# alessandroragano/nomad

Hardware: NVIDIA B200
Metric: utterance-seconds embedded per second (higher is better)
Workload: dtype fp16

## Files before the change

### nomad_b200/csrc/gemm.cu

```cuda
#include "gemm.cuh"

#include <cmath>
#include <cstdlib>
#include <cstring>
#include <mutex>
#include <vector>

namespace nb {

static constexpr int BM = 128;
static constexpr int BK = 64;
static constexpr int UMMA_K = 16;
static constexpr int NUM_EPI_WARPS = 8;
static constexpr int GEMM_THREADS = 128 + NUM_EPI_WARPS * 32;
static constexpr float CD_REFINE = 1e-3f;

template <int BN>
struct TileCfg {
    static constexpr int A_BYTES = BM * BK * 2;
    static constexpr int B_BYTES = BN * BK * 2;
    static constexpr int STAGE_BYTES = A_BYTES + B_BYTES;
    static constexpr int STAGES = (BN == 256) ? 4 : (BN == 192 ? 4 : (BN == 128 ? 5 : 7));
    static constexpr int ACC_STRIDE = BN <= 64 ? 64 : (BN <= 128 ? 128 : 256);
    static constexpr int TMEM_COLS = 2 * ACC_STRIDE;
    static constexpr int EPI_STAGE_BYTES = NUM_EPI_WARPS * 4096;
    static constexpr int SMEM_BYTES = STAGES * STAGE_BYTES + EPI_STAGE_BYTES + 1024  + 256 ;
};

struct GemmArgs {
    int M, N, K, batch;
    int umma_n;
    int m_tiles, n_tiles;
    int a_wrap;
    int shared_ab, b_kshift0, b_kshift_step, b_mod;
    int resid_tma;
    int resid_l2pf;
    unsigned sleep_ns;
    GemmEpilogue epi;
};
__device__ __forceinline__ void mbar_wait_role(uint64_t* bar, uint32_t parity, unsigned ns) {
    if (mbar_try_wait(bar, parity)) return;
    while (!mbar_try_wait(bar, parity))
        if (ns) __nanosleep(ns);
}

struct RowCtx {
    float2 st;
    float pm, pM2;
    float* rbuf;
    bool rhave;
    const float* rnext;
    const CUtensorMap* tm_r;
    uint64_t* rbar;
    uint32_t rphase;
    const float* rbase;
    const float* vec;
    int vec_stride;
    int vec_col0;
    const CUtensorMap* tm_f;
    const CUtensorMap* tm_h;
    const CUtensorMap* tm_a;
    uint32_t pending;
    int stage_bytes;
    int flip;
};
__device__ __forceinline__ void resid_tma_issue(const CUtensorMap* map, uint64_t* bar, float* rbuf, const float* src,
                                                const float* base, long long ld, int lane) {
    if (lane == 0) {
        const long long off = src - base;
        const int row = (int)(off / ld), col = (int)(off - (long long)row * ld);
        mbar_expect_tx(bar, 4096);
        tma_load_2d_cta(rbuf, map, bar, col, row);
    }
}
__device__ __forceinline__ void ts_acquire(RowCtx& rc, uint32_t mask, int lane) {
    if (rc.pending & mask) {
        if (lane == 0) bulk_wait_read();
        rc.pending = 0;
    }
    __syncwarp();
    rc.pending |= mask;
}
__device__ __forceinline__ void ts_issue(const CUtensorMap* map, const void* src, int col, long long row, int lane) {
    fence_proxy_async_smem();
    __syncwarp();
    if (lane == 0) {
        tma_store_2d(map, src, col, (int)row);
        bulk_commit();
    }
}
__device__ __forceinline__ int ts_h16_slot(RowCtx& rc, bool f32_too) {
    if (rc.stage_bytes >= 6144) return 4096;
    if (f32_too) return 0;
    rc.flip ^= 1;
    return rc.flip * 2048;
}
__device__ __forceinline__ float2 ln_row_stats(const float* part, long long row) {
    const float4* p = reinterpret_cast<const float4*>(part + row * (2 * LN_PARTS));
    float m[LN_PARTS], M2 = 0.f, mean = 0.f;
#pragma unroll
    for (int i = 0; i < LN_PARTS / 2; ++i) {
        const float4 t = __ldg(p + i);
        m[2 * i] = t.x; m[2 * i + 1] = t.z;
        M2 += t.y + t.w;
        mean += t.x + t.z;
    }
    mean *= 1.0f / LN_PARTS;
    float d2 = 0.f;
#pragma unroll
    for (int i = 0; i < LN_PARTS; ++i) d2 = fmaf(m[i] - mean, m[i] - mean, d2);
    const float var = fmaf(64.0f, d2, M2) * (1.0f / (64.0f * LN_PARTS));
    return make_float2(mean, rsqrtf(var + 1e-5f));
}

template <int EF>
__device__ __forceinline__ int epi_flags(const GemmEpilogue& e) { return EF >= 0 ? EF : e.flags; }

template <int EF>
__device__ __forceinline__ float2 epilogue_row_stats(const GemmArgs& args, long long row) {
    if (row >= args.M || !(epi_flags<EF>(args.epi) & (EPI_LN_FOLD | EPI_RESID_LN))) return make_float2(0.f, 1.f);
    return args.epi.ln_part != nullptr ? ln_row_stats(args.epi.ln_part, row)
                                       : __ldg(reinterpret_cast<const float2*>(args.epi.ln_stats) + row);
}

template <int EF, int W>
__device__ __forceinline__ void epilogue_stage_vectors(const GemmEpilogue& e, float* vec, int c0, int lane) {
    const int flags = epi_flags<EF>(e);
    __syncwarp();
    if (lane * 4 < W) {
        if (flags & EPI_BIAS) reinterpret_cast<float4*>(vec)[lane] = __ldg(reinterpret_cast<const float4*>(e.bias + c0) + lane);
        if (flags & EPI_LN_FOLD) {
            reinterpret_cast<float4*>(vec)[lane] = __ldg(reinterpret_cast<const float4*>(e.fold_c + c0) + lane);
            reinterpret_cast<float4*>(vec + W)[lane] = __ldg(reinterpret_cast<const float4*>(e.fold_s + c0) + lane);
        }
        if (flags & EPI_RESID_LN) {
            reinterpret_cast<float4*>(vec + W)[lane] = __ldg(reinterpret_cast<const float4*>(e.ln_g + c0) + lane);
            reinterpret_cast<float4*>(vec + 2 * W)[lane] = __ldg(reinterpret_cast<const float4*>(e.ln_b + c0) + lane);
        }
    }
    __syncwarp();
}

template <bool FULL, int EF, bool PREC = false, bool TS = false, bool SV = false, bool RP = false>
__device__ __forceinline__ void epilogue_chunk(const GemmEpilogue& e, float (&v)[32], long long row, bool row_ok,
                                               int rows_valid, int col0, int ncols, int b, float* stage, int lane,
                                               RowCtx& rc) {
    const int flags = epi_flags<EF>(e);
    const long long off = row * e.ldo + col0 + (long long)b * e.out_bstride;
    const long long woff = (row - lane) * e.ldo + col0 + (long long)b * e.out_bstride;
    if (PREC) {
        const float sc = e.acc_scale;
#pragma unroll
        for (int j = 0; j < 32; ++j) v[j] *= sc;
    }
    if ((FULL || row_ok) && (flags & EPI_BIAS)) {
        const float4* bp = reinterpret_cast<const float4*>(e.bias + (long long)b * e.bias_bstride + col0);
#pragma unroll
        for (int j = 0; j < 8; ++j) {
            if (FULL || j * 4 < ncols) {
                const float4 t = (FULL && (SV || rc.vec)) ? *reinterpret_cast<const float4*>(rc.vec + (col0 - rc.vec_col0) + 4 * j)
                                                          : __ldg(bp + j);
                v[4 * j + 0] += t.x; v[4 * j + 1] += t.y; v[4 * j + 2] += t.z; v[4 * j + 3] += t.w;
            }
        }
    }
    if ((FULL || row_ok) && (flags & EPI_LN_FOLD)) {
        const float4* sp = reinterpret_cast<const float4*>(e.fold_s + col0);
        const float4* cp = reinterpret_cast<const float4*>(e.fold_c + col0);
        const float nm = -rc.st.x, rs = rc.st.y;
#pragma unroll
        for (int j = 0; j < 8; ++j) {
            if (FULL || j * 4 < ncols) {
                const bool sv = FULL && (SV || rc.vec != nullptr);
                const float4 a = sv ? *reinterpret_cast<const float4*>(rc.vec + rc.vec_stride + (col0 - rc.vec_col0) + 4 * j)
                                    : __ldg(sp + j);
                const float4 c = sv ? *reinterpret_cast<const float4*>(rc.vec + (col0 - rc.vec_col0) + 4 * j) : __ldg(cp + j);
#if NB_F32X2
                const float2 nm2 = make_float2(nm, nm), rs2 = make_float2(rs, rs);
                const float2 lo = ffma2(rs2, ffma2(nm2, make_float2(a.x, a.y), make_float2(v[4 * j + 0], v[4 * j + 1])), make_float2(c.x, c.y));
                const float2 hi = ffma2(rs2, ffma2(nm2, make_float2(a.z, a.w), make_float2(v[4 * j + 2], v[4 * j + 3])), make_float2(c.z, c.w));
                v[4 * j + 0] = lo.x; v[4 * j + 1] = lo.y; v[4 * j + 2] = hi.x; v[4 * j + 3] = hi.y;
#else
// ... 211 lines not shown
        for (int j = 0; j < 32; ++j) nbv[j] = j < ncols ? __ldg(e.norm_b + col0 + j) : 0.f;
    }
    const float m2s = -2.0f * e.cd_inv_scale;
    float dmin = CD_REFINE;
#pragma unroll
    for (int j = 0; j < 32; ++j) {
        v[j] = fmaf(v[j], m2s, na + nbv[j]);
        if (full || j < ncols) dmin = fminf(dmin, v[j]);
    }
    if (row_ok && dmin < CD_REFINE) {
#pragma unroll
        for (int j = 0; j < 32; ++j)
            if (j < ncols && v[j] < CD_REFINE) v[j] = cdist_exact_d2(e.cd_a + row * 256, e.cd_b + (long long)(col0 + j) * 256);
    }
    float s4[4] = {0.f, 0.f, 0.f, 0.f};
#pragma unroll
    for (int j = 0; j < 32; ++j) {
        v[j] = sqrt_approx(fmaxf(v[j], 0.f));
        if (full || j < ncols) s4[j & 3] += v[j];
    }
    s32 = (s4[0] + s4[1]) + (s4[2] + s4[3]);
    const double rs = row_ok ? (double)s32 : 0.0;
    if (e.out_f != nullptr && ts != nullptr && ts->tm_f != nullptr) {
        ts->flip ^= 1;
        float* sp = stage + (ts->stage_bytes >= 8192 ? ts->flip * 1024 : 0);
        ts_acquire(*ts, ts->stage_bytes >= 8192 ? (3u << (2 * ts->flip)) : 3u, lane);
        stage_put_f32(sp, v, lane);
        ts_issue(ts->tm_f, sp, col0, row - lane, lane);
    } else if (e.out_f != nullptr) {
        stage_put_f32(stage, v, lane);
        float* wout = e.out_f + (row - lane) * e.ldo + col0;
        if (full && (e.ldo & 3) == 0 && ((reinterpret_cast<uintptr_t>(wout) & 15) == 0)) {
            stage_flush_f32(stage, wout, e.ldo, rows_valid, ncols, lane);
        } else {
            __syncwarp();
            for (int rl = 0; rl < 32 && rl < rows_valid; ++rl)
                if (lane < ncols) wout[rl * e.ldo + lane] = stage[rl * 32 + ((((lane >> 2) ^ (rl & 7)) << 2) | (lane & 3))];
            __syncwarp();
        }
    }
    return rs;
}

struct StoreMaps {
    const CUtensorMap *f, *h, *a;
    const CUtensorMap* r;
    uint64_t* rbar;
    uint32_t* rphase;
    int stage_bytes;
    uint32_t* pending;
    int* flip;
};

template <int CHUNKS, bool PAIR, bool CDIST, int EF, bool PREC = false, int PACC = 0, bool TS = false, bool SV = false, bool RP = false>
__device__ __forceinline__ void epilogue_tile(const GemmArgs& args, uint32_t taddr, long long row, int col_first,
                                              int ccol_first, int b, uint64_t* tmem_empty_bar, int lane, float* stage,
                                              float2 row_st, float* rbuf, bool& rhave, const float* next_tile_src,
                                              const float* vec = nullptr, int vec_stride = 0, int cd_group = 0,
                                              const StoreMaps* sm = nullptr) {
    const bool row_ok = row < args.M;
    const long long rv = (long long)args.M - (row - lane);
    const int rows_valid = rv > 32 ? 32 : (rv < 0 ? 0 : (int)rv);
    double row_sum = 0.0;
    RowCtx rc;
    rc.st = row_st;
    rc.pm = rc.pM2 = 0.f;
    rc.rbuf = rbuf;
    rc.rhave = rhave;
    rc.rnext = nullptr;
    rc.vec = vec;
    rc.vec_stride = vec_stride;
    rc.vec_col0 = col_first;
    rc.tm_f = rc.tm_h = rc.tm_a = nullptr;
    rc.tm_r = nullptr; rc.rbar = nullptr; rc.rphase = 0; rc.rbase = args.epi.resid;
    if (sm != nullptr && sm->r != nullptr) { rc.tm_r = sm->r; rc.rbar = sm->rbar; rc.rphase = *sm->rphase; }
    rc.pending = 0;
    rc.stage_bytes = 4096;
    rc.flip = 0;
    if (TS && sm != nullptr) {
        rc.tm_f = sm->f; rc.tm_h = sm->h; rc.tm_a = sm->a;
        rc.stage_bytes = sm->stage_bytes;
        rc.pending = *sm->pending;
        rc.flip = *sm->flip;
    }
#pragma unroll 1
    for (int c = 0; c < CHUNKS; ++c) {
        uint32_t r[32];
        tmem_ld_32x32(taddr + c * 32, r);
        tmem_ld_wait();
        if (PREC && PACC > 0) {
#pragma unroll 1
            for (int a = 1; a < 4; ++a) {
                uint32_t q[32];
                tmem_ld_32x32(taddr + a * PACC + c * 32, q);
                tmem_ld_wait();
#pragma unroll
                for (int j = 0; j < 32; ++j) r[j] = __float_as_uint(__uint_as_float(r[j]) + __uint_as_float(q[j]));
            }
        }
        if (c == CHUNKS - 1) {
            tc_fence_before();
            __syncwarp();
            if (lane == 0) {
                if (PAIR) mbar_arrive_cluster(tmem_empty_bar, 0); else mbar_arrive(tmem_empty_bar);
            }
        }
        const int col0 = col_first + c * 32;
        int ncols = args.N - col0;
        ncols = ncols > 32 ? 32 : ncols;
        if (ccol_first + c * 32 >= args.umma_n) ncols = 0;
        if (!CDIST && rbuf != nullptr) {
            rc.rnext = next_tile_src;
            if (c + 1 < CHUNKS) {
                const int col1 = col0 + 32;
                rc.rnext = (rows_valid == 32 && col1 + 32 <= args.N && ccol_first + (c + 1) * 32 + 32 <= args.umma_n)
                               ? args.epi.resid + (row - lane) * args.epi.ldr + col1
                               : nullptr;
            }
        }
        if (ncols > 0 && rows_valid > 0) {
            float v[32];
#pragma unroll
            for (int j = 0; j < 32; ++j) v[j] = __uint_as_float(r[j]);
            if (CDIST) row_sum += cdist_chunk(args.epi, v, row, row_ok, rows_valid, col0, ncols, stage, lane, TS ? &rc : nullptr);
            else if (rows_valid == 32 && ncols == 32) epilogue_chunk<true, EF, PREC, TS, SV, RP>(args.epi, v, row, true, 32, col0, 32, b, stage, lane, rc);
            else epilogue_chunk<false, EF, PREC, TS>(args.epi, v, row, row_ok, rows_valid, col0, ncols, b, stage, lane, rc);
        }
    }
    rhave = rc.rhave;
    if (sm != nullptr && sm->r != nullptr) *sm->rphase = rc.rphase;
    if (TS && sm != nullptr) {
        *sm->pending = rc.pending;
        *sm->flip = rc.flip;
    }
    if (CDIST && row_ok) args.epi.row_part[(long long)cd_group * args.M + row] = (float)row_sum;
}

template <int BN, bool CDIST, bool PREC = false>
__global__ void __launch_bounds__(GEMM_THREADS, 1)
gemm_tc_kernel(const __grid_constant__ CUtensorMap tmA, const __grid_constant__ CUtensorMap tmB,
               const __grid_constant__ CUtensorMap tmA2, const __grid_constant__ CUtensorMap tmB2, const GemmArgs args) {
    using Cfg = TileCfg<BN>;
    constexpr int STAGES = Cfg::STAGES;
    extern __shared__ uint8_t smem_raw[];
    uint8_t* smem = smem_raw + ((1024u - (smem_u32(smem_raw) & 1023u)) & 1023u);
    float* epi_stage = reinterpret_cast<float*>(smem + STAGES * Cfg::STAGE_BYTES);
    uint64_t* full_bar = reinterpret_cast<uint64_t*>(smem + STAGES * Cfg::STAGE_BYTES + Cfg::EPI_STAGE_BYTES);
    uint64_t* empty_bar = full_bar + STAGES;
    uint64_t* tmem_full = empty_bar + STAGES;
    uint64_t* tmem_empty = tmem_full + 2;
    uint32_t* tmem_slot = reinterpret_cast<uint32_t*>(tmem_empty + 2);

    const int warp = threadIdx.x >> 5;
    const int lane = threadIdx.x & 31;
    const int num_tiles = args.m_tiles * args.n_tiles * args.batch;
    const int k_blocks = (args.K + BK - 1) / BK;
    const int k_total = PREC ? 3 * k_blocks : k_blocks;

    if (warp == 0 && lane == 0) {
        tma_prefetch_desc(&tmA);
        tma_prefetch_desc(&tmB);
    }
    if (warp == 1 && lane == 0) {
        for (int s = 0; s < STAGES; ++s) {
            mbar_init(&full_bar[s], 1);
            mbar_init(&empty_bar[s], 1);
// ... 45 lines not shown
            }
        }
    } else if (warp == 1) {
        if (lane == 0) {
            const uint32_t idesc = umma_idesc_h16(BM, args.umma_n);
            int stage = 0;
            uint32_t phase = 0;
            int it = 0;
            for (int tile = blockIdx.x; tile < num_tiles; tile += gridDim.x, ++it) {
                const int as = PREC ? 0 : (it & 1);
                const uint32_t aphase = PREC ? (it & 1) : ((it >> 1) & 1);
                mbar_wait_role(&tmem_empty[as], aphase ^ 1, args.sleep_ns);
                tc_fence_after();
                uint32_t started = 0;
                for (int kb = 0; kb < k_total; ++kb) {
                    mbar_wait_role(&full_bar[stage], phase, args.sleep_ns);
                    tc_fence_after();
                    const uint32_t sa = smem_u32(smem + stage * Cfg::STAGE_BYTES);
                    const uint32_t sb = sa + Cfg::A_BYTES;
                    const uint64_t da = umma_desc_sw128(sa);
                    const uint64_t db = umma_desc_sw128(sb);
                    const int acc = PREC ? (kb < k_blocks ? kb % 3 : 3) : as;
                    const uint32_t d_tmem = tmem_base + acc * Cfg::ACC_STRIDE;
                    const uint32_t cont = PREC ? ((started >> acc) & 1u) : (kb ? 1u : 0u);
                    started |= 1u << acc;
#pragma unroll
                    for (int k = 0; k < BK / UMMA_K; ++k) {
                        umma_f16(d_tmem, da + (uint64_t)(2 * k), db + (uint64_t)(2 * k), idesc, (cont | k) ? 1u : 0u);
                    }
                    umma_commit(&empty_bar[stage]);
                    if (kb == k_total - 1) umma_commit(&tmem_full[as]);
                    if (++stage == STAGES) { stage = 0; phase ^= 1; }
                }
            }
        }
    } else if (warp >= 4) {
        const int ew = warp - 4;
        const int q = warp & 3;
        const int h = ew >> 2;
        constexpr int HALF = BN / 2;
        constexpr int CHUNKS = (HALF + 31) / 32;
        bool no_prefetch = false;
        int it = 0;
        for (int tile = blockIdx.x; tile < num_tiles; tile += gridDim.x, ++it) {
            const int n_blk = tile % args.n_tiles;
            const int m_blk = (tile / args.n_tiles) % args.m_tiles;
            const int b = tile / (args.n_tiles * args.m_tiles);
            const int as = PREC ? 0 : (it & 1);
            const uint32_t aphase = PREC ? (it & 1) : ((it >> 1) & 1);
            const long long row = (long long)m_blk * BM + q * 32 + lane;
            const float2 row_st = CDIST ? make_float2(0.f, 1.f) : epilogue_row_stats<-1>(args, row);
            mbar_wait(&tmem_full[as], aphase);
            tc_fence_after();
            epilogue_tile<CHUNKS, false, CDIST, -1, PREC, Cfg::ACC_STRIDE>(args, tmem_base + (uint32_t)(as * Cfg::ACC_STRIDE + h * HALF) + ((uint32_t)(q * 32) << 16),
                                         row, n_blk * BN + h * HALF, h * HALF, b, &tmem_empty[as], lane, epi_stage + ew * 1024,
                                         row_st, nullptr, no_prefetch, nullptr, nullptr, 0, n_blk * 2 + h);
        }
    }
    tc_fence_before();
    __syncthreads();
    if (warp == 2) {
        tc_fence_after();
        tmem_dealloc(tmem_base, TCOLS);
    }
}

struct Pair256 {
    static constexpr int BN = 256;
    static constexpr int A_BYTES = BM * BK * 2;
    static constexpr int B_BYTES = (BN / 2) * BK * 2;
    static constexpr int STAGE_BYTES = A_BYTES + B_BYTES;
    static constexpr int STAGES = 5;
    static constexpr int resid_bytes(int epi_warps, bool rpf) { return rpf ? epi_warps * 4096 : 0; }
    static constexpr int vec_bytes(int epi_warps) { return epi_warps * 3 * (BN / (epi_warps / 4)) * 4; }
    static constexpr int stages(int epi_warps, bool rpf) { return 4; }
    static constexpr int stage_bytes(int epi_warps, bool cdist) { return (epi_warps == 8 && !cdist) ? 6144 : 4096; }
    static constexpr int smem_bytes(int epi_warps, bool rpf, bool cdist = false) {
        return stages(epi_warps, rpf) * STAGE_BYTES + epi_warps * stage_bytes(epi_warps, cdist) + resid_bytes(epi_warps, rpf) +
               vec_bytes(epi_warps) + 1024 + 256;
    }
};

template <int NEW, bool CDIST, bool RPF, int EF, bool PREC = false, bool TS = false>
__global__ void __cluster_dims__(2, 1, 1) __launch_bounds__(128 + 32 * NEW, 1)
gemm_tc_pair_kernel(const __grid_constant__ CUtensorMap tmA, const __grid_constant__ CUtensorMap tmB,
                    const __grid_constant__ CUtensorMap tmA2, const __grid_constant__ CUtensorMap tmB2,
                    const __grid_constant__ CUtensorMap tmOutF, const __grid_constant__ CUtensorMap tmOutH,
                    const __grid_constant__ CUtensorMap tmAux, const __grid_constant__ CUtensorMap tmResid, const GemmArgs args) {
    using Cfg = Pair256;
    constexpr int STAGES = Cfg::stages(NEW, RPF);
    constexpr int BN = Cfg::BN;
    extern __shared__ uint8_t smem_raw[];
    uint8_t* smem = smem_raw + ((1024u - (smem_u32(smem_raw) & 1023u)) & 1023u);
    float* epi_stage = reinterpret_cast<float*>(smem + STAGES * Cfg::STAGE_BYTES);
    constexpr int SB = Cfg::stage_bytes(NEW, CDIST);
    constexpr bool SPEC = !CDIST && EF >= 0;
    constexpr bool SPEC_SV = SPEC && (EF & (EPI_BIAS | EPI_LN_FOLD | EPI_RESID_LN)) != 0;
    float* resid_stage = reinterpret_cast<float*>(smem + STAGES * Cfg::STAGE_BYTES + NEW * SB);
    float* vec_stage = reinterpret_cast<float*>(smem + STAGES * Cfg::STAGE_BYTES + NEW * SB + Cfg::resid_bytes(NEW, RPF));
    uint64_t* full_bar = reinterpret_cast<uint64_t*>(smem + STAGES * Cfg::STAGE_BYTES + NEW * SB + Cfg::resid_bytes(NEW, RPF) +
                                                     Cfg::vec_bytes(NEW));
    uint64_t* empty_bar = full_bar + STAGES;
    uint64_t* tmem_full = empty_bar + STAGES;
    uint64_t* tmem_empty = tmem_full + 2;
    uint64_t* resid_bar = tmem_empty + 2;
    uint32_t* tmem_slot = reinterpret_cast<uint32_t*>(resid_bar + NEW);

    const int warp = threadIdx.x >> 5;
    const int lane = threadIdx.x & 31;
    const uint32_t rank = cluster_ctarank();
    const bool leader = rank == 0;
    const int pair_id = blockIdx.x >> 1, num_pairs = gridDim.x >> 1;
    const int num_tiles = args.m_tiles * args.n_tiles * args.batch;
    const int k_blocks = (args.K + BK - 1) / BK;
    const int k_total = PREC ? 3 * k_blocks : k_blocks;

    if (warp == 0 && lane == 0) {
        tma_prefetch_desc(&tmA);
        tma_prefetch_desc(&tmB);
    }
    if (warp == 1 && lane == 0) {
        for (int s = 0; s < STAGES; ++s) {
            mbar_init(&full_bar[s], 1);
            mbar_init(&empty_bar[s], 1);
        }
        for (int s = 0; s < 2; ++s) {
            mbar_init(&tmem_full[s], 1);
            mbar_init(&tmem_empty[s], 2 * NEW);
        }
        for (int s = 0; s < NEW; ++s) mbar_init(&resid_bar[s], 1);
        mbar_fence_init();
    }
    if (warp == 2) {
        tmem_alloc_pair(tmem_slot, 512);
        tmem_relinquish_pair();
    }
    tc_fence_before();
    cluster_sync_all();
    tc_fence_after();
    const uint32_t tmem_base = *tmem_slot;
    asm volatile("griddepcontrol.wait;" ::: "memory");
    asm volatile("griddepcontrol.launch_dependents;" ::: "memory");

    if (warp == 0) {
        if (lane == 0) {
            int stage = 0;
            uint32_t phase = 0;
            for (int tile = pair_id; tile < num_tiles; tile += num_pairs) {
                const int n_blk = tile % args.n_tiles;
                const int m_blk = (tile / args.n_tiles) % args.m_tiles;
                const int b = tile / (args.n_tiles * args.m_tiles);
                const int row0 = m_blk * 256 + (int)rank * BM;
                const int col0 = n_blk * BN + (int)rank * (BN / 2);
                for (int kq = 0; kq < k_total; ++kq) {
                    const int seg = PREC ? kq / k_blocks : 0, kb = PREC ? kq - seg * k_blocks : kq;
                    const CUtensorMap* mA = (PREC && seg == 1) ? &tmA2 : &tmA;
                    const CUtensorMap* mB = (PREC && seg == 2) ? &tmB2 : &tmB;
                    mbar_wait_role(&empty_bar[stage], phase ^ 1, args.sleep_ns);
                    uint8_t* sa = smem + stage * Cfg::STAGE_BYTES;
                    uint8_t* sb = sa + Cfg::A_BYTES;
                    if (leader) mbar_expect_tx(&full_bar[stage], 2 * Cfg::STAGE_BYTES);
                    if (args.a_wrap > 0) {
                        const int kk = kb * BK;
                        tma_load_3d_pair(sa, mA, &full_bar[stage], kk % args.a_wrap, row0 + kk / args.a_wrap, b);
                    } else {
                        tma_load_3d_pair(sa, mA, &full_bar[stage], kb * BK, row0, b);
                    }
                    tma_load_3d_pair(sb, mB, &full_bar[stage], kb * BK, col0, b);
                    if (++stage == STAGES) { stage = 0; phase ^= 1; }
                }
            }
        }
    } else if (warp == 1) {
        if (lane == 0 && leader) {
            const uint32_t idesc = umma_idesc_h16(256, BN);
            int stage = 0;
            uint32_t phase = 0;
            int it = 0;
            for (int tile = pair_id; tile < num_tiles; tile += num_pairs, ++it) {
                const int as = it & 1;
                const uint32_t aphase = (it >> 1) & 1;
                mbar_wait_role(&tmem_empty[as], aphase ^ 1, args.sleep_ns);
                tc_fence_after();
                const uint32_t d_tmem = tmem_base + as * 256;
                for (int kb = 0; kb < k_total; ++kb) {
                    mbar_wait_role(&full_bar[stage], phase, args.sleep_ns);
                    tc_fence_after();
                    const uint32_t sa = smem_u32(smem + stage * Cfg::STAGE_BYTES);
                    const uint64_t da = umma_desc_sw128(sa);
                    const uint64_t db = umma_desc_sw128(sa + Cfg::A_BYTES);
#pragma unroll
                    for (int k = 0; k < BK / UMMA_K; ++k)
                        umma_f16_pair(d_tmem, da + (uint64_t)(2 * k), db + (uint64_t)(2 * k), idesc, (kb | k) ? 1u : 0u);
                    umma_commit_pair(&empty_bar[stage]);
                    if (kb == k_total - 1) umma_commit_pair(&tmem_full[as]);
                    if (++stage == STAGES) { stage = 0; phase ^= 1; }
                }
            }
        }
    } else if (warp >= 4) {
        const int ew = warp - 4;
        const int q = warp & 3;
        const int h = ew >> 2;
        constexpr int HALF = BN / (NEW / 4);
        const int eflags = epi_flags<EF>(args.epi);
        const bool want_pf = RPF && (eflags & (EPI_RESID | EPI_RESID_LN)) != 0 && args.batch == 1;
        float* rbuf = want_pf ? resid_stage + ew * 1024 : nullptr;
        auto tile_src = [&](int t) -> const float* {
            if (!want_pf || t >= num_tiles) return nullptr;
            const int n2 = t % args.n_tiles, m2 = (t / args.n_tiles) % args.m_tiles;
            const long long r0 = (long long)m2 * 256 + rank * BM + q * 32;
            const int c0 = n2 * BN + h * HALF;
            return (r0 + 32 <= args.M && c0 + 32 <= args.N) ? args.epi.resid + r0 * args.epi.ldr + c0 : nullptr;
        };
        uint32_t ts_pending = 0;
        int ts_flip = 0;
        StoreMaps smaps;
        smaps.f = (TS && (eflags & (EPI_OUT_F32 | EPI_CDIST)) && args.epi.out_f != nullptr) ? &tmOutF : nullptr;
        smaps.h = (TS && (eflags & EPI_OUT_H16)) ? &tmOutH : nullptr;
        smaps.a = (TS && (eflags & EPI_SAVE_DGELU)) ? &tmAux : nullptr;
        smaps.stage_bytes = SB;
        smaps.pending = &ts_pending;
        smaps.flip = &ts_flip;
        uint32_t rphase = 0;
        smaps.r = (want_pf && args.resid_tma) ? &tmResid : nullptr;
        smaps.rbar = &resid_bar[ew];
        smaps.rphase = &rphase;
        bool rhave = false;
        if (want_pf) {
            const float* src = tile_src(pair_id);
            if (src != nullptr) {
                if (smaps.r != nullptr) resid_tma_issue(smaps.r, smaps.rbar, rbuf, src, args.epi.resid, args.epi.ldr, lane);
                else stage_fill_f32_async(rbuf, src, args.epi.ldr, lane);
                rhave = true;
            }
        }
        int it = 0;
        for (int tile = pair_id; tile < num_tiles; tile += num_pairs, ++it) {
            const int n_blk = tile % args.n_tiles;
            const int m_blk = (tile / args.n_tiles) % args.m_tiles;
            const int b = tile / (args.n_tiles * args.m_tiles);
            const int as = it & 1;
            const uint32_t aphase = (it >> 1) & 1;
            const long long row = (long long)m_blk * 256 + rank * BM + q * 32 + lane;
            const float2 row_st = CDIST ? make_float2(0.f, 1.f) : epilogue_row_stats<EF>(args, row);
            if (!CDIST && (!want_pf || args.resid_l2pf > 0) && (eflags & (EPI_RESID | EPI_RESID_LN)) &&
                tile + (want_pf ? args.resid_l2pf : 1) * num_pairs < num_tiles) {
                const int nt = tile + (want_pf ? args.resid_l2pf : 1) * num_pairs;
                const int n2 = nt % args.n_tiles, m2 = (nt / args.n_tiles) % args.m_tiles;
                const long long r2 = (long long)m2 * 256 + rank * BM + q * 32 + lane;
                const int c2 = n2 * BN + h * HALF;
                if (r2 < args.M && c2 + HALF <= args.N)
                    prefetch_l2_bulk(args.epi.resid + r2 * args.epi.ldr + c2, HALF * 4);
            }
            const float* next_src = tile_src(tile + num_pairs);
            float* vec = nullptr;
            if (!CDIST && args.batch == 1 && n_blk * BN + h * HALF + HALF <= args.N &&
                (eflags & (EPI_BIAS | EPI_LN_FOLD | EPI_RESID_LN)) != 0) {
                vec = vec_stage + ew * (3 * HALF);
                epilogue_stage_vectors<EF, HALF>(args.epi, vec, n_blk * BN + h * HALF, lane);
            }
            mbar_wait(&tmem_full[as], aphase);
            tc_fence_after();
            epilogue_tile<HALF / 32, true, CDIST, EF, PREC, 0, TS, SPEC_SV, SPEC && RPF && (EF & (EPI_RESID | EPI_RESID_LN)) != 0>(args, tmem_base + (uint32_t)(as * 256 + h * HALF) + ((uint32_t)(q * 32) << 16), row,
                                           n_blk * BN + h * HALF, h * HALF, b, &tmem_empty[as], lane, epi_stage + ew * (SB / 4),
                                           row_st, rbuf, rhave, next_src, vec, HALF, n_blk * (NEW / 4) + h, &smaps);
        }
        if (TS && lane == 0) bulk_wait_all();
    }
    tc_fence_before();
    cluster_sync_all();
    if (warp == 2) {
        tc_fence_after();
        tmem_dealloc_pair(tmem_base, 512);
    }
}

__global__ void gemm_simt_kernel(GemmOperand A, GemmOperand B, GemmArgs args) {
    __shared__ float sa[16][17];
    __shared__ float sb[16][17];
    const int b = blockIdx.z;
    const long long row = (long long)blockIdx.y * 16 + threadIdx.y;
    const int col = blockIdx.x * 16 + threadIdx.x;
    const op_t* a = A.ptr + (long long)b * A.batch_stride;
    const op_t* w = B.ptr + (long long)b * B.batch_stride;
    float acc = 0.f;
    for (int k0 = 0; k0 < args.K; k0 += 16) {
        const long long ar = (long long)blockIdx.y * 16 + threadIdx.y;
        const int ak = k0 + threadIdx.x;
        const long long aoff = A.k_wrap > 0 ? (ar + ak / A.k_wrap) * A.row_stride + ak % A.k_wrap : ar * A.row_stride + ak;
        sa[threadIdx.y][threadIdx.x] = (ar < args.M && ak < args.K) ? op2f(a[aoff]) : 0.f;
        const int br = blockIdx.x * 16 + threadIdx.y;
        sb[threadIdx.y][threadIdx.x] = (br < args.N && ak < args.K) ? op2f(w[(long long)br * B.row_stride + ak]) : 0.f;
        __syncthreads();
#pragma unroll
        for (int k = 0; k < 16; ++k) acc = fmaf(sa[threadIdx.y][k], sb[threadIdx.x][k], acc);
        __syncthreads();
    }
    if (row < args.M && col < args.N) epilogue_scalar(args.epi, acc, row, col, b);
}

typedef CUresult (*EncodeTiledFn)(CUtensorMap*, CUtensorMapDataType, cuuint32_t, void*, const cuuint64_t*,
                                  const cuuint64_t*, const cuuint32_t*, const cuuint32_t*, CUtensorMapInterleave,
                                  CUtensorMapSwizzle, CUtensorMapL2promotion, CUtensorMapFloatOOBfill);

static EncodeTiledFn get_encode_fn() {
    static EncodeTiledFn fn = nullptr;
    static std::once_flag once;
    std::call_once(once, [] {
        void* p = nullptr;
        cudaDriverEntryPointQueryResult qres;
        if (cudaGetDriverEntryPoint("cuTensorMapEncodeTiled", &p, cudaEnableDefault, &qres) == cudaSuccess &&
            qres == cudaDriverEntryPointSuccess)
            fn = reinterpret_cast<EncodeTiledFn>(p);
    });
    return fn;
}

static int make_operand_map(CUtensorMap* map, const GemmOperand& op, int K, int batch, int box_rows) {
// ... 137 lines not shown
    return (args.epi.flags & EPI_CDIST) ? launch_tc_impl<BN, true>(st, A, B, args) : launch_tc_impl<BN, false>(st, A, B, args);
}

static int make_store_map(CUtensorMap* map, const void* ptr, bool f32, long long rows, long long cols, long long ld) {
    EncodeTiledFn fn = get_encode_fn();
    NB_CHECK(fn != nullptr, "cuTensorMapEncodeTiled is not available from the CUDA driver");
    const size_t el = f32 ? 4 : 2;
    cuuint64_t gdim[2] = {(cuuint64_t)cols, (cuuint64_t)rows};
    cuuint64_t gstride[1] = {(cuuint64_t)ld * el};
    cuuint32_t box[2] = {32, 32};
    cuuint32_t estr[2] = {1, 1};
    CUresult r = fn(map, f32 ? CU_TENSOR_MAP_DATA_TYPE_FLOAT32 : CU_TENSOR_MAP_DATA_TYPE_FLOAT16, 2, const_cast<void*>(ptr), gdim,
                    gstride, box, estr, CU_TENSOR_MAP_INTERLEAVE_NONE, f32 ? CU_TENSOR_MAP_SWIZZLE_128B : CU_TENSOR_MAP_SWIZZLE_64B,
                    CU_TENSOR_MAP_L2_PROMOTION_NONE, CU_TENSOR_MAP_FLOAT_OOB_FILL_NONE);
    NB_CHECK(r == CUDA_SUCCESS, "cuTensorMapEncodeTiled (store map) failed (%d): rows=%lld cols=%lld ld=%lld", (int)r, rows, cols, ld);
    return 0;
}
static bool tma_store_ok(const GemmArgs& args) {
    static const int enabled = getenv("NOMAD_B200_TMA_STORE") ? atoi(getenv("NOMAD_B200_TMA_STORE")) : 1;
    const GemmEpilogue& e = args.epi;
    if (!enabled || args.batch != 1 || (e.flags & EPI_PRECISE)) return false;
    if (enabled == 1 && ((e.flags & (EPI_RESID | EPI_RESID_LN | EPI_SAVE_DGELU | EPI_MUL_AUX)) ||
                         ((e.flags & EPI_LN_FOLD) && (e.flags & EPI_GELU))))
        return false;
    auto ok = [&](const void* p, size_t el) { return p != nullptr && ((uintptr_t)p & 15) == 0 && (e.ldo * el) % 16 == 0; };
    if ((e.flags & EPI_CDIST) && e.out_f != nullptr && !ok(e.out_f, 4)) return false;
    if ((e.flags & EPI_OUT_F32) && !ok(e.out_f, 4)) return false;
    if ((e.flags & EPI_OUT_H16) && !ok(e.out_h, 2)) return false;
    if ((e.flags & EPI_SAVE_DGELU) && !ok(e.aux_out, 2)) return false;
    return true;
}

template <int NEW, bool CDIST, bool RPF = false, int EF = -1, bool PREC = false, bool TS = true>
static int launch_pair_impl(cudaStream_t st, const GemmOperand& A, const GemmOperand& B, GemmArgs& args) {
    using Cfg = Pair256;
    if (TS && !tma_store_ok(args)) return launch_pair_impl<NEW, CDIST, RPF, EF, PREC, false>(st, A, B, args);
    constexpr int SMEM = Cfg::smem_bytes(NEW, RPF, CDIST);
    static bool attr_set[64] = {false};
    if (bool* flag = device_once_flag(attr_set)) {
        NB_CUDA(cudaFuncSetAttribute(gemm_tc_pair_kernel<NEW, CDIST, RPF, EF, PREC, TS>, cudaFuncAttributeMaxDynamicSharedMemorySize, SMEM));
        *flag = true;
    }
    CUtensorMap tmA, tmB, tmA2, tmB2;
    NB_TRY(make_operand_map(&tmA, A, args.K, args.batch, BM));
    NB_TRY(make_operand_map(&tmB, B, args.K, args.batch, Cfg::BN / 2));
    GemmOperand Al, Bl;
    lo_operand(A, &Al);
    lo_operand(B, &Bl);
    NB_TRY(make_operand_map(&tmA2, Al, args.K, args.batch, BM));
    NB_TRY(make_operand_map(&tmB2, Bl, args.K, args.batch, Cfg::BN / 2));
    args.umma_n = Cfg::BN;
    args.m_tiles = (args.M + 255) / 256;
    args.n_tiles = (args.N + Cfg::BN - 1) / Cfg::BN;
    const long long tiles = (long long)args.m_tiles * args.n_tiles * args.batch;
    int pairs = device_sm_count() / 2;
    if (tiles < pairs) pairs = (int)tiles;
    NB_TRY(prof_begin(st, 2.0 * args.M * args.N * args.K * args.batch));
    CUtensorMap tmF = tmA, tmH = tmA, tmX = tmA, tmR = tmA;
    if (RPF && args.resid_tma) NB_TRY(make_store_map(&tmR, args.epi.resid, true, args.M, args.N, args.epi.ldr));
    if (TS) {
        const GemmEpilogue& e = args.epi;
        if ((e.flags & (EPI_OUT_F32 | EPI_CDIST)) && e.out_f) NB_TRY(make_store_map(&tmF, e.out_f, true, args.M, args.N, e.ldo));
        if (e.flags & EPI_OUT_H16) NB_TRY(make_store_map(&tmH, e.out_h, false, args.M, args.N, e.ldo));
        if (e.flags & EPI_SAVE_DGELU) NB_TRY(make_store_map(&tmX, e.aux_out, false, args.M, args.N, e.ldo));
    }
    static const int pdl = getenv("NOMAD_B200_PDL") ? atoi(getenv("NOMAD_B200_PDL")) : 1;
    if (pdl) {
        cudaLaunchConfig_t cfg;
        memset(&cfg, 0, sizeof(cfg));
        cfg.gridDim = dim3(2 * pairs);
        cfg.blockDim = dim3(128 + 32 * NEW);
        cfg.dynamicSmemBytes = SMEM;
        cfg.stream = st;
        cudaLaunchAttribute attr[1];
        attr[0].id = cudaLaunchAttributeProgrammaticStreamSerialization;
        attr[0].val.programmaticStreamSerializationAllowed = 1;
        cfg.attrs = attr;
        cfg.numAttrs = 1;
        NB_CUDA(cudaLaunchKernelEx(&cfg, gemm_tc_pair_kernel<NEW, CDIST, RPF, EF, PREC, TS>, tmA, tmB, tmA2, tmB2, tmF, tmH, tmX, tmR, args));
    } else {
        gemm_tc_pair_kernel<NEW, CDIST, RPF, EF, PREC, TS><<<2 * pairs, 128 + 32 * NEW, SMEM, st>>>(tmA, tmB, tmA2, tmB2, tmF, tmH, tmX, tmR, args);
    }
    NB_LAUNCHED();
    NB_TRY(prof_end(st));
    return 0;
}
static int launch_pair(cudaStream_t st, const GemmOperand& A, const GemmOperand& B, GemmArgs& args) {
    if (args.epi.flags & EPI_CDIST) return launch_pair_impl<16, true>(st, A, B, args);
    static const int epi16 = getenv("NOMAD_B200_EPI16") ? atoi(getenv("NOMAD_B200_EPI16")) : 1;
    const int fl = args.epi.flags;
    const bool heavy = args.K <= 1024 && ((fl & (EPI_GELU | EPI_SAVE_DGELU)) != 0 ||
                                          ((fl & (EPI_RESID | EPI_RESID_LN)) != 0 && !(fl & EPI_STATS_OUT)));
    static const int spec_env = getenv("NOMAD_B200_EPI_SPEC") ? atoi(getenv("NOMAD_B200_EPI_SPEC")) : 1;
    const bool spec = spec_env && args.N % Pair256::BN == 0 && args.batch == 1;
    constexpr int F_FC1 = EPI_LN_FOLD | EPI_GELU | EPI_OUT_H16;
    constexpr int F_QKV = EPI_LN_FOLD | EPI_OUT_H16;
    constexpr int F_CONV = EPI_GELU | EPI_OUT_H16;
    constexpr int F_RES = EPI_BIAS | EPI_RESID_LN | EPI_OUT_F32 | EPI_OUT_H16 | EPI_STATS_OUT;
    constexpr int F_FC1_SAVE = EPI_BIAS | EPI_GELU | EPI_OUT_H16 | EPI_SAVE_DGELU;
    constexpr int F_CONV_SAVE = EPI_GELU | EPI_OUT_H16 | EPI_SAVE_DGELU;
    constexpr int F_LIN_H16 = EPI_BIAS | EPI_OUT_H16;
    constexpr int F_RES_PLAIN = EPI_BIAS | EPI_RESID_LN | EPI_OUT_F32;
    constexpr int F_BRES = EPI_BIAS | EPI_RESID | EPI_OUT_F32;
    constexpr int F_DG_RES = EPI_RESID | EPI_OUT_F32;
    constexpr int F_DG_AUX = EPI_MUL_AUX | EPI_OUT_H16;
    constexpr int F_H16 = EPI_OUT_H16;
    if (epi16 == 2 || (epi16 == 1 && heavy)) {
        if (spec && fl == F_BRES) return launch_pair_impl<16, false, false, F_BRES>(st, A, B, args);
        if (spec && fl == F_RES_PLAIN) return launch_pair_impl<16, false, false, F_RES_PLAIN>(st, A, B, args);
        if (spec && fl == F_FC1) return launch_pair_impl<16, false, false, F_FC1>(st, A, B, args);
        if (spec && fl == F_CONV) return launch_pair_impl<16, false, false, F_CONV>(st, A, B, args);
        if (spec && fl == F_FC1_SAVE) return launch_pair_impl<16, false, false, F_FC1_SAVE>(st, A, B, args);
        if (spec && fl == F_CONV_SAVE) return launch_pair_impl<16, false, false, F_CONV_SAVE>(st, A, B, args);
        return launch_pair_impl<16, false>(st, A, B, args);
    }
    static const int rpf = getenv("NOMAD_B200_RESID_PREFETCH") ? atoi(getenv("NOMAD_B200_RESID_PREFETCH")) : 1;
    if (rpf && (fl & (EPI_RESID | EPI_RESID_LN)) != 0 && args.batch == 1) {
        if (spec && fl == F_RES) return launch_pair_impl<8, false, true, F_RES>(st, A, B, args);
        if (spec && fl == F_RES_PLAIN) return launch_pair_impl<8, false, true, F_RES_PLAIN>(st, A, B, args);
        if (spec && fl == F_BRES) return launch_pair_impl<8, false, true, F_BRES>(st, A, B, args);
        if (spec && fl == F_DG_RES) return launch_pair_impl<8, false, true, F_DG_RES>(st, A, B, args);
        return launch_pair_impl<8, false, true>(st, A, B, args);
    }
    if (spec && fl == F_QKV) return launch_pair_impl<8, false, false, F_QKV>(st, A, B, args);
    if (spec && fl == F_CONV) return launch_pair_impl<8, false, false, F_CONV>(st, A, B, args);
    if (spec && fl == F_CONV_SAVE) return launch_pair_impl<8, false, false, F_CONV_SAVE>(st, A, B, args);
    if (spec && fl == F_LIN_H16) return launch_pair_impl<8, false, false, F_LIN_H16>(st, A, B, args);
    if (spec && fl == F_DG_AUX) return launch_pair_impl<8, false, false, F_DG_AUX>(st, A, B, args);
    if (spec && fl == F_H16) return launch_pair_impl<8, false, false, F_H16>(st, A, B, args);
    return launch_pair_impl<8, false>(st, A, B, args);
}

static thread_local int g_corr_shift0 = 0, g_corr_step = 0, g_corr_on = 0, g_corr_mod = 1;

int gemm_h16_corr(cudaStream_t st, const GemmOperand& A, const GemmOperand& B, int M, int N, int K, int batch, int shift0,
                  int step, int b_mod, const GemmEpilogue& epi) {
    NB_CHECK(N <= 128, "gemm_h16_corr: N <= 128");
    NB_CHECK(shift0 % 8 == 0 && step % 8 == 0 && b_mod >= 1, "gemm_h16_corr: shifts must be multiples of 8 elements");
    g_corr_on = 1; g_corr_shift0 = shift0; g_corr_step = step; g_corr_mod = b_mod;
    const int rc = gemm_h16(st, A, B, M, N, K, batch, epi, 0);
    g_corr_on = 0;
    return rc;
}

int gemm_h16(cudaStream_t st, const GemmOperand& A, const GemmOperand& B, int M, int N, int K, int batch,
              const GemmEpilogue& epi, int impl) {
    if (M <= 0 || N <= 0 || batch <= 0) return 0;
    NB_CHECK(K > 0 && K % 8 == 0, "GEMM K=%d must be a positive multiple of 8", K);
    GemmArgs args;
    args.M = M; args.N = N; args.K = K; args.batch = batch;
    args.epi = epi;
    args.umma_n = 0; args.m_tiles = args.n_tiles = 0;
    args.a_wrap = A.k_wrap;
    args.shared_ab = g_corr_on; args.b_kshift0 = g_corr_shift0; args.b_kshift_step = g_corr_step; args.b_mod = g_corr_mod;
    static const unsigned sleep_ns = getenv("NOMAD_B200_GEMM_SLEEP") ? (unsigned)atoi(getenv("NOMAD_B200_GEMM_SLEEP")) : 0u;
    args.sleep_ns = sleep_ns;
    static const int resid_l2pf = getenv("NOMAD_B200_RESID_L2PF") ? atoi(getenv("NOMAD_B200_RESID_L2PF")) : 0;
    args.resid_l2pf = resid_l2pf;
    static const int resid_tma = getenv("NOMAD_B200_RESID_TMA") ? atoi(getenv("NOMAD_B200_RESID_TMA")) : 0;
    args.resid_tma = (resid_tma && (epi.flags & (EPI_RESID | EPI_RESID_LN)) && epi.resid != nullptr && batch == 1 &&
                      ((uintptr_t)epi.resid & 15) == 0 && (epi.ldr * 4) % 16 == 0) ? 1 : 0;
    NB_CHECK(B.k_wrap == 0, "only the A operand may use wrapped K");
    if (epi.flags & EPI_PRECISE) {
        NB_CHECK(impl == 0 && A.lo != nullptr && B.lo != nullptr && epi.acc_scale > 0.f, "EPI_PRECISE needs hi + lo operand planes and a scale");
        NB_CHECK(!(epi.flags & EPI_OUT_H16) || epi.out_l != nullptr, "EPI_PRECISE with a 16-bit output needs the lo plane pointer");
        NB_CHECK(!(epi.flags & (EPI_CDIST | EPI_LN_FOLD | EPI_STATS_OUT | EPI_RESID_LN | EPI_SAVE_DGELU | EPI_MUL_AUX)),
                 "EPI_PRECISE supports bias / GELU / residual / fp32 and split 16-bit outputs only");
    }
    if (!(epi.flags & EPI_CDIST)) {
        NB_CHECK(N % 8 == 0 && epi.ldo % 8 == 0 && epi.out_bstride % 8 == 0,
                 "GEMM epilogue needs N, ldo, out_bstride multiples of 8 (N=%d ldo=%lld bstride=%lld)", N, epi.ldo,
                 epi.out_bstride);
        NB_CHECK(!(epi.flags & EPI_RESID) || (epi.ldr % 4 == 0 && epi.resid_bstride % 4 == 0),
                 "GEMM residual leading dimension must be a multiple of 4");
    }
    NB_CHECK(!(epi.flags & (EPI_LN_FOLD | EPI_STATS_OUT)) || impl == 0, "LayerNorm-folding epilogues exist only in the tensor-core kernel");
    NB_CHECK(!(epi.flags & EPI_STATS_OUT) || (N == 64 * LN_PARTS && batch == 1 && epi.part_out != nullptr),
             "EPI_STATS_OUT needs N = %d", 64 * LN_PARTS);
    NB_CHECK(!(epi.flags & EPI_LN_FOLD) || (epi.ln_part && epi.fold_s && epi.fold_c && N % 4 == 0 && batch == 1),
             "EPI_LN_FOLD needs partial statistics, s and c vectors");
    if (impl == 1) {
        dim3 grid((N + 15) / 16, (M + 15) / 16, batch), block(16, 16);
        gemm_simt_kernel<<<grid, block, 0, st>>>(A, B, args);
        NB_LAUNCHED();
        return 0;
    }
    if (epi.flags & EPI_PRECISE) {
        NB_CHECK(K >= 3 * BK, "EPI_PRECISE needs K >= %d", 3 * BK);
        if (N > 64) {
            args.umma_n = 128;
            return launch_tc<128>(st, A, B, args);
        }
        args.umma_n = (N + 15) / 16 * 16;
        return launch_tc<64>(st, A, B, args);
    }
    if (use_pair_kernel(M, N, batch)) return launch_pair(st, A, B, args);
    if (N > 128) {
        static const int force_bn = getenv("NOMAD_B200_BN") ? atoi(getenv("NOMAD_B200_BN")) : 0;
        const double sms = device_sm_count();
        auto eff = [&](int bn, double tile_eff) {
            const double tiles = (double)((M + BM - 1) / BM) * ((N + bn - 1) / bn) * batch;
            const double used = (double)N / (((N + bn - 1) / bn) * (double)bn);
            return tile_eff * used * tiles / (std::ceil(tiles / sms) * sms);
        };
        const bool use192 = (epi.flags & (EPI_STATS_OUT | EPI_CDIST | EPI_PRECISE)) ? false : (force_bn ? force_bn == 192 : eff(192, 0.89) > eff(256, 1.0));
// ... 17 lines not shown
```

Before: 57600.

## Split tail-wave pair GEMM tiles into narrower N pieces to fill idle SMs

In the 2-CTA pair GEMM, the tiles left over after the last full wave are split into 64- or 128-column pieces so more SM pairs get work in the tail. It adds a second B tensor map for the narrower width, a per-item UMMA instruction descriptor, and a runtime chunk count in the epilogue, including an early TMEM-empty arrive for epilogue groups that have no columns. The aim is to cut wave-quantization idle time. In exchange, narrower MMAs reuse the A operand less per load, and the item-indexing arithmetic costs a little more.

```diff
diff --git a/nomad_b200/csrc/gemm.cu b/nomad_b200/csrc/gemm.cu
--- a/nomad_b200/csrc/gemm.cu
+++ b/nomad_b200/csrc/gemm.cu
@@ -36,6 +36,7 @@
     int resid_tma;
     int resid_l2pf;
     unsigned sleep_ns;
+    int items, full_tiles, piece_w;
     GemmEpilogue epi;
 };
 __device__ __forceinline__ void mbar_wait_role(uint64_t* bar, uint32_t parity, unsigned ns) {
@@ -124,10 +125,10 @@
 }
 
 template <int EF, int W>
-__device__ __forceinline__ void epilogue_stage_vectors(const GemmEpilogue& e, float* vec, int c0, int lane) {
+__device__ __forceinline__ void epilogue_stage_vectors(const GemmEpilogue& e, float* vec, int c0, int n, int lane) {
     const int flags = epi_flags<EF>(e);
     __syncwarp();
-    if (lane * 4 < W) {
+    if (lane * 4 < n) {
         if (flags & EPI_BIAS) reinterpret_cast<float4*>(vec)[lane] = __ldg(reinterpret_cast<const float4*>(e.bias + c0) + lane);
         if (flags & EPI_LN_FOLD) {
             reinterpret_cast<float4*>(vec)[lane] = __ldg(reinterpret_cast<const float4*>(e.fold_c + c0) + lane);
@@ -445,8 +446,8 @@
     int* flip;
 };
 
-template <int CHUNKS, bool PAIR, bool CDIST, int EF, bool PREC = false, int PACC = 0, bool TS = false, bool SV = false, bool RP = false>
-__device__ __forceinline__ void epilogue_tile(const GemmArgs& args, uint32_t taddr, long long row, int col_first,
+template <bool PAIR, bool CDIST, int EF, bool PREC = false, int PACC = 0, bool TS = false, bool SV = false, bool RP = false>
+__device__ __forceinline__ void epilogue_tile(const GemmArgs& args, int nch, uint32_t taddr, long long row, int col_first,
                                               int ccol_first, int b, uint64_t* tmem_empty_bar, int lane, float* stage,
                                               float2 row_st, float* rbuf, bool& rhave, const float* next_tile_src,
                                               const float* vec = nullptr, int vec_stride = 0, int cd_group = 0,
@@ -476,8 +477,15 @@
         rc.pending = *sm->pending;
         rc.flip = *sm->flip;
     }
+    if (nch == 0) {
+        tc_fence_before();
+        __syncwarp();
+        if (lane == 0) {
+            if (PAIR) mbar_arrive_cluster(tmem_empty_bar, 0); else mbar_arrive(tmem_empty_bar);
+        }
+    }
 #pragma unroll 1
-    for (int c = 0; c < CHUNKS; ++c) {
+    for (int c = 0; c < nch; ++c) {
         uint32_t r[32];
         tmem_ld_32x32(taddr + c * 32, r);
         tmem_ld_wait();
@@ -491,7 +499,7 @@
                 for (int j = 0; j < 32; ++j) r[j] = __float_as_uint(__uint_as_float(r[j]) + __uint_as_float(q[j]));
             }
         }
-        if (c == CHUNKS - 1) {
+        if (c == nch - 1) {
             tc_fence_before();
             __syncwarp();
             if (lane == 0) {
@@ -504,7 +512,7 @@
         if (ccol_first + c * 32 >= args.umma_n) ncols = 0;
         if (!CDIST && rbuf != nullptr) {
             rc.rnext = next_tile_src;
-            if (c + 1 < CHUNKS) {
+            if (c + 1 < nch) {
                 const int col1 = col0 + 32;
                 rc.rnext = (rows_valid == 32 && col1 + 32 <= args.N && ccol_first + (c + 1) * 32 + 32 <= args.umma_n)
                                ? args.epi.resid + (row - lane) * args.epi.ldr + col1
@@ -656,7 +664,7 @@
             const float2 row_st = CDIST ? make_float2(0.f, 1.f) : epilogue_row_stats<-1>(args, row);
             mbar_wait(&tmem_full[as], aphase);
             tc_fence_after();
-            epilogue_tile<CHUNKS, false, CDIST, -1, PREC, Cfg::ACC_STRIDE>(args, tmem_base + (uint32_t)(as * Cfg::ACC_STRIDE + h * HALF) + ((uint32_t)(q * 32) << 16),
+            epilogue_tile<false, CDIST, -1, PREC, Cfg::ACC_STRIDE>(args, CHUNKS, tmem_base + (uint32_t)(as * Cfg::ACC_STRIDE + h * HALF) + ((uint32_t)(q * 32) << 16),
                                          row, n_blk * BN + h * HALF, h * HALF, b, &tmem_empty[as], lane, epi_stage + ew * 1024,
                                          row_st, nullptr, no_prefetch, nullptr, nullptr, 0, n_blk * 2 + h);
         }
@@ -685,12 +693,38 @@
     }
 };
 
+struct PairItem {
+    int m_blk, b;
+    int col0, w;
+};
+template <bool CUT>
+__device__ __forceinline__ PairItem pair_item(const GemmArgs& args, int i) {
+    int t = i, sub = 0, w = Pair256::BN;
+    if (CUT && i >= args.full_tiles) {
+        const int per = Pair256::BN / args.piece_w;
+        t = args.full_tiles + (i - args.full_tiles) / per;
+        sub = (i - args.full_tiles) % per;
+        w = args.piece_w;
+    }
+    PairItem p;
+    p.m_blk = (t / args.n_tiles) % args.m_tiles;
+    p.b = t / (args.n_tiles * args.m_tiles);
+    p.col0 = (t % args.n_tiles) * Pair256::BN + sub * w;
+    p.w = w;
+    return p;
+}
+__device__ __forceinline__ int pair_group_cols(int w, int groups, bool stats) {
+    const int c = w / groups, lo = stats ? 64 : 32;
+    return c < lo ? lo : c;
+}
+
 template <int NEW, bool CDIST, bool RPF, int EF, bool PREC = false, bool TS = false>
 __global__ void __cluster_dims__(2, 1, 1) __launch_bounds__(128 + 32 * NEW, 1)
 gemm_tc_pair_kernel(const __grid_constant__ CUtensorMap tmA, const __grid_constant__ CUtensorMap tmB,
                     const __grid_constant__ CUtensorMap tmA2, const __grid_constant__ CUtensorMap tmB2,
                     const __grid_constant__ CUtensorMap tmOutF, const __grid_constant__ CUtensorMap tmOutH,
-                    const __grid_constant__ CUtensorMap tmAux, const __grid_constant__ CUtensorMap tmResid, const GemmArgs args) {
+                    const __grid_constant__ CUtensorMap tmAux, const __grid_constant__ CUtensorMap tmResid,
+                    const __grid_constant__ CUtensorMap tmBn, const GemmArgs args) {
     using Cfg = Pair256;
     constexpr int STAGES = Cfg::stages(NEW, RPF);
     constexpr int BN = Cfg::BN;
@@ -715,7 +749,8 @@
     const uint32_t rank = cluster_ctarank();
     const bool leader = rank == 0;
     const int pair_id = blockIdx.x >> 1, num_pairs = gridDim.x >> 1;
-    const int num_tiles = args.m_tiles * args.n_tiles * args.batch;
+    const int num_items = args.items;
+    constexpr bool CUT = !CDIST && !PREC;
     const int k_blocks = (args.K + BK - 1) / BK;
     const int k_total = PREC ? 3 * k_blocks : k_blocks;
 
@@ -750,20 +785,21 @@
         if (lane == 0) {
             int stage = 0;
             uint32_t phase = 0;
-            for (int tile = pair_id; tile < num_tiles; tile += num_pairs) {
-                const int n_blk = tile % args.n_tiles;
-                const int m_blk = (tile / args.n_tiles) % args.m_tiles;
-                const int b = tile / (args.n_tiles * args.m_tiles);
-                const int row0 = m_blk * 256 + (int)rank * BM;
-                const int col0 = n_blk * BN + (int)rank * (BN / 2);
+            for (int i = pair_id; i < num_items; i += num_pairs) {
+                const PairItem p = pair_item<CUT>(args, i);
+                const int b = p.b;
+                const int row0 = p.m_blk * 256 + (int)rank * BM;
+                const int col0 = p.col0 + (int)rank * (p.w / 2);
+                const CUtensorMap* mBw = p.w == BN ? &tmB : &tmBn;
+                const uint32_t tx_bytes = 2 * Cfg::A_BYTES + (uint32_t)p.w * BK * 2;
                 for (int kq = 0; kq < k_total; ++kq) {
                     const int seg = PREC ? kq / k_blocks : 0, kb = PREC ? kq - seg * k_blocks : kq;
                     const CUtensorMap* mA = (PREC && seg == 1) ? &tmA2 : &tmA;
-                    const CUtensorMap* mB = (PREC && seg == 2) ? &tmB2 : &tmB;
+                    const CUtensorMap* mB = (PREC && seg == 2) ? &tmB2 : mBw;
                     mbar_wait_role(&empty_bar[stage], phase ^ 1, args.sleep_ns);
                     uint8_t* sa = smem + stage * Cfg::STAGE_BYTES;
                     uint8_t* sb = sa + Cfg::A_BYTES;
-                    if (leader) mbar_expect_tx(&full_bar[stage], 2 * Cfg::STAGE_BYTES);
+                    if (leader) mbar_expect_tx(&full_bar[stage], tx_bytes);
                     if (args.a_wrap > 0) {
                         const int kk = kb * BK;
                         tma_load_3d_pair(sa, mA, &full_bar[stage], kk % args.a_wrap, row0 + kk / args.a_wrap, b);
@@ -777,11 +813,11 @@
         }
     } else if (warp == 1) {
         if (lane == 0 && leader) {
-            const uint32_t idesc = umma_idesc_h16(256, BN);
             int stage = 0;
             uint32_t phase = 0;
             int it = 0;
-            for (int tile = pair_id; tile < num_tiles; tile += num_pairs, ++it) {
+            for (int i = pair_id; i < num_items; i += num_pairs, ++it) {
+                const uint32_t idesc = umma_idesc_h16(256, pair_item<CUT>(args, i).w);
                 const int as = it & 1;
                 const uint32_t aphase = (it >> 1) & 1;
                 mbar_wait_role(&tmem_empty[as], aphase ^ 1, args.sleep_ns);
@@ -808,13 +844,16 @@
         const int h = ew >> 2;
         constexpr int HALF = BN / (NEW / 4);
         const int eflags = epi_flags<EF>(args.epi);
+        const bool stats = (eflags & EPI_STATS_OUT) != 0;
         const bool want_pf = RPF && (eflags & (EPI_RESID | EPI_RESID_LN)) != 0 && args.batch == 1;
         float* rbuf = want_pf ? resid_stage + ew * 1024 : nullptr;
         auto tile_src = [&](int t) -> const float* {
-            if (!want_pf || t >= num_tiles) return nullptr;
-            const int n2 = t % args.n_tiles, m2 = (t / args.n_tiles) % args.m_tiles;
-            const long long r0 = (long long)m2 * 256 + rank * BM + q * 32;
-            const int c0 = n2 * BN + h * HALF;
+            if (!want_pf || t >= num_items) return nullptr;
+            const PairItem p2 = pair_item<CUT>(args, t);
+            const int cc = h * pair_group_cols(p2.w, NEW / 4, stats);
+            if (cc >= p2.w) return nullptr;
+            const long long r0 = (long long)p2.m_blk * 256 + rank * BM + q * 32;
+            const int c0 = p2.col0 + cc;
             return (r0 + 32 <= args.M && c0 + 32 <= args.N) ? args.epi.resid + r0 * args.epi.ldr + c0 : nullptr;
         };
         uint32_t ts_pending = 0;
@@ -840,35 +879,38 @@
             }
         }
         int it = 0;
-        for (int tile = pair_id; tile < num_tiles; tile += num_pairs, ++it) {
-            const int n_blk = tile % args.n_tiles;
-            const int m_blk = (tile / args.n_tiles) % args.m_tiles;
-            const int b = tile / (args.n_tiles * args.m_tiles);
+        for (int i = pair_id; i < num_items; i += num_pairs, ++it) {
+            const PairItem p = pair_item<CUT>(args, i);
+            const int b = p.b;
+            const int gcols = pair_group_cols(p.w, NEW / 4, stats);
+            const int ccol = h * gcols;
+            const int nch = ccol < p.w ? gcols / 32 : 0;
+            const int col_first = p.col0 + ccol;
             const int as = it & 1;
             const uint32_t aphase = (it >> 1) & 1;
-            const long long row = (long long)m_blk * 256 + rank * BM + q * 32 + lane;
+            const long long row = (long long)p.m_blk * 256 + rank * BM + q * 32 + lane;
             const float2 row_st = CDIST ? make_float2(0.f, 1.f) : epilogue_row_stats<EF>(args, row);
             if (!CDIST && (!want_pf || args.resid_l2pf > 0) && (eflags & (EPI_RESID | EPI_RESID_LN)) &&
-                tile + (want_pf ? args.resid_l2pf : 1) * num_pairs < num_tiles) {
-                const int nt = tile + (want_pf ? args.resid_l2pf : 1) * num_pairs;
-                const int n2 = nt % args.n_tiles, m2 = (nt / args.n_tiles) % args.m_tiles;
-                const long long r2 = (long long)m2 * 256 + rank * BM + q * 32 + lane;
-                const int c2 = n2 * BN + h * HALF;
-                if (r2 < args.M && c2 + HALF <= args.N)
-                    prefetch_l2_bulk(args.epi.resid + r2 * args.epi.ldr + c2, HALF * 4);
-            }
-            const float* next_src = tile_src(tile + num_pairs);
+                i + (want_pf ? args.resid_l2pf : 1) * num_pairs < num_items) {
+                const PairItem p2 = pair_item<CUT>(args, i + (want_pf ? args.resid_l2pf : 1) * num_pairs);
+                const int g2 = pair_group_cols(p2.w, NEW / 4, stats);
+                const long long r2 = (long long)p2.m_blk * 256 + rank * BM + q * 32 + lane;
+                const int c2 = p2.col0 + h * g2;
+                if (h * g2 < p2.w && r2 < args.M && c2 + g2 <= args.N)
+                    prefetch_l2_bulk(args.epi.resid + r2 * args.epi.ldr + c2, g2 * 4);
+            }
+            const float* next_src = tile_src(i + num_pairs);
             float* vec = nullptr;
-            if (!CDIST && args.batch == 1 && n_blk * BN + h * HALF + HALF <= args.N &&
+            if (!CDIST && args.batch == 1 && nch > 0 && col_first + gcols <= args.N &&
                 (eflags & (EPI_BIAS | EPI_LN_FOLD | EPI_RESID_LN)) != 0) {
                 vec = vec_stage + ew * (3 * HALF);
-                epilogue_stage_vectors<EF, HALF>(args.epi, vec, n_blk * BN + h * HALF, lane);
+                epilogue_stage_vectors<EF, HALF>(args.epi, vec, col_first, gcols, lane);
             }
             mbar_wait(&tmem_full[as], aphase);
             tc_fence_after();
-            epilogue_tile<HALF / 32, true, CDIST, EF, PREC, 0, TS, SPEC_SV, SPEC && RPF && (EF & (EPI_RESID | EPI_RESID_LN)) != 0>(args, tmem_base + (uint32_t)(as * 256 + h * HALF) + ((uint32_t)(q * 32) << 16), row,
-                                           n_blk * BN + h * HALF, h * HALF, b, &tmem_empty[as], lane, epi_stage + ew * (SB / 4),
-                                           row_st, rbuf, rhave, next_src, vec, HALF, n_blk * (NEW / 4) + h, &smaps);
+            epilogue_tile<true, CDIST, EF, PREC, 0, TS, SPEC_SV, SPEC && RPF && (EF & (EPI_RESID | EPI_RESID_LN)) != 0>(args, nch, tmem_base + (uint32_t)(as * 256 + ccol) + ((uint32_t)(q * 32) << 16), row,
+                                           col_first, ccol, b, &tmem_empty[as], lane, epi_stage + ew * (SB / 4),
+                                           row_st, rbuf, rhave, next_src, vec, HALF, (p.col0 / BN) * (NEW / 4) + h, &smaps);
         }
         if (TS && lane == 0) bulk_wait_all();
     }
@@ -1112,9 +1154,21 @@
     args.umma_n = Cfg::BN;
     args.m_tiles = (args.M + 255) / 256;
     args.n_tiles = (args.N + Cfg::BN - 1) / Cfg::BN;
-    const long long tiles = (long long)args.m_tiles * args.n_tiles * args.batch;
-    int pairs = device_sm_count() / 2;
-    if (tiles < pairs) pairs = (int)tiles;
+    const int tiles = args.m_tiles * args.n_tiles * args.batch;
+    const int max_pairs = device_sm_count() / 2;
+    const int rest = tiles % max_pairs;
+    args.full_tiles = tiles - rest;
+    args.piece_w = Cfg::BN;
+    if (!CDIST && !PREC && rest > 0)
+        for (int w : {64, 128})
+            if (rest * (Cfg::BN / w) <= max_pairs) {
+                args.piece_w = w;
+                break;
+            }
+    args.items = args.full_tiles + rest * (Cfg::BN / args.piece_w);
+    const int pairs = args.items < max_pairs ? args.items : max_pairs;
+    CUtensorMap tmBn = tmB;
+    if (args.piece_w < Cfg::BN) NB_TRY(make_operand_map(&tmBn, B, args.K, args.batch, args.piece_w / 2));
     NB_TRY(prof_begin(st, 2.0 * args.M * args.N * args.K * args.batch));
     CUtensorMap tmF = tmA, tmH = tmA, tmX = tmA, tmR = tmA;
     if (RPF && args.resid_tma) NB_TRY(make_store_map(&tmR, args.epi.resid, true, args.M, args.N, args.epi.ldr));
@@ -1137,9 +1191,9 @@
         attr[0].val.programmaticStreamSerializationAllowed = 1;
         cfg.attrs = attr;
         cfg.numAttrs = 1;
-        NB_CUDA(cudaLaunchKernelEx(&cfg, gemm_tc_pair_kernel<NEW, CDIST, RPF, EF, PREC, TS>, tmA, tmB, tmA2, tmB2, tmF, tmH, tmX, tmR, args));
+        NB_CUDA(cudaLaunchKernelEx(&cfg, gemm_tc_pair_kernel<NEW, CDIST, RPF, EF, PREC, TS>, tmA, tmB, tmA2, tmB2, tmF, tmH, tmX, tmR, tmBn, args));
     } else {
-        gemm_tc_pair_kernel<NEW, CDIST, RPF, EF, PREC, TS><<<2 * pairs, 128 + 32 * NEW, SMEM, st>>>(tmA, tmB, tmA2, tmB2, tmF, tmH, tmX, tmR, args);
+        gemm_tc_pair_kernel<NEW, CDIST, RPF, EF, PREC, TS><<<2 * pairs, 128 + 32 * NEW, SMEM, st>>>(tmA, tmB, tmA2, tmB2, tmF, tmH, tmX, tmR, tmBn, args);
     }
     NB_LAUNCHED();
     NB_TRY(prof_end(st));
@@ -1211,6 +1265,7 @@
     args.M = M; args.N = N; args.K = K; args.batch = batch;
     args.epi = epi;
     args.umma_n = 0; args.m_tiles = args.n_tiles = 0;
+    args.items = args.full_tiles = 0; args.piece_w = 256;
     args.a_wrap = A.k_wrap;
     args.shared_ab = g_corr_on; args.b_kshift0 = g_corr_shift0; args.b_kshift_step = g_corr_step; args.b_mod = g_corr_mod;
     static const unsigned sleep_ns = getenv("NOMAD_B200_GEMM_SLEEP") ? (unsigned)atoi(getenv("NOMAD_B200_GEMM_SLEEP")) : 0u;
```

New measurement: 56810 (median of 6 runs). 1.4% lower.
